# FrancisGregoryNg/Gaussian_Process_Optimization

Hardware: AMD Instinct MI355X
Metric: GP fit+predict iters/sec at N=16384 D=8 (higher is better)
Workload: dtype f64; 1 GPU; C3 (BASELINE.json configs[2]): N=16384, D=8 RBF iso, fit (K, Cholesky, alpha, LML) + predict mean/var at M=10000 candidates + EI arg-best; candidates_total=10000, candidates_this_rank=10000, entry_point=gp_fit_predict, kernel=RBF, fit=replicated on every rank (does not shard, SURVEY.md 8e), torch_imported=False, launcher=single process, emulate_fp64=0

## Files before the change

### gaussian_process_optimization_amd/csrc/api_factor.hip

```cpp
#include "api_internal.h"

void build_ky(gp_ctx *g, const Members &m, bool jittered) {
    launch_kbuild(g->s, m.A, m.lda, m.X, g->N, g->Npad, m.kp[0], m.diag[0], 0, m.nb, m.sA, m.kpt, m.diag_tab, m.sX);
    if (jittered) launch_add_diag(g->s, m.A, m.lda, g->N, m.jit[0], m.nb, m.sA, m.jit_tab);
    launch_set_rhs(g->s, m.A, m.lda, m.Y, g->N, g->Npad, g->P, m.nb, m.sA, m.sY);
}

static int chain_step(gp_ctx *g, hipStream_t s, const Members &m, int j, int J1, int R1) {
    double *A = m.A, *invL = m.invL;
    const long lda = m.lda;
    if (g->inner_tiles >= 2 && m.nb == 1 && j + 1 < J1 && R1 - (j + 2) >= g->inner_min_rows) {
        launch_potrf_pair(s, A, lda, j, invL, m.info);
        launch_trsm2(s, A, lda, j, invL, j + 2, R1);
        if (j + 2 < J1)
            gemm(g, s, 1, A, lda, A + (long)j * GP_TILE, lda, A + (long)j * GP_TILE, lda, 1, 2 * GP_TILE,
                 TileSet{0, R1, j + 2, J1, 1});
        return j + 2;
    }
    launch_potrf_tile(s, A, lda, j, invL, m.info, m.nb, m.sA, m.sI, 4);
    gemm(g, s, 0, A, lda, A + (long)j * GP_TILE, lda, invL + (long)j * GP_TILE * GP_TILE, GP_TILE, 0, GP_TILE,
         TileSet{j + 1, R1, j, j + 1, 0}, member_opt(m, inplace_opt(), m.sA, m.sA, m.sI));
    if (j + 1 < J1)
        gemm(g, s, 1, A, lda, A + (long)j * GP_TILE, lda, A + (long)j * GP_TILE, lda, 1, GP_TILE, TileSet{0, R1, j + 1, J1, 1},
             member_opt(m, GemmOpt(), m.sA, m.sA, m.sA));
// ... 126 lines not shown
        if (Gf == 1) {
            rlaunch(sb, J, J1, J2, p.nt, J == 0 ? 1 : 0);
            rebuild_next(J);
            GP_NOTE(hipEventRecord(la_event(g, EV_BULK, J), sb));
            return;
        }
        const int gi = J / Gf, Jg = gi * Gf;
        const int first = gi == 0 ? 1 : 0;
        GP_NOTE(hipEventRecord(la_event(g, EV_CONV, J), sb));
        rlaunch(sb, Jg, J1, p.edge(J + 2), p.edge(J + 3), first);
        rebuild_next(J);
        GP_NOTE(hipEventRecord(la_event(g, EV_BULK, J), sb));
        if (J % Gf == Gf - 1) {
            if (gi >= 1 && far_issued[gi - 1]) GP_NOTE(hipStreamWaitEvent(sb, la_event(g, EV_FAR, gi - 1), 0));
            mid_Jg = Jg;
            mid_end = J1;
            mid_first = first;
            mid_base = J + 3;
            mid_next = 0;
            if (p.edge(J + 3 + Gf) < p.nt) {
                GP_NOTE(hipStreamWaitEvent(sfar, la_event(g, EV_CONV, J), 0));
                rlaunch(sfar, Jg, J1, p.edge(J + 3 + Gf), p.nt, first);
                GP_NOTE(hipEventRecord(la_event(g, EV_FAR, gi), sfar));
                far_issued[gi] = true;
            }
        }
        if (mid_Jg >= 0 && mid_next < Gf) {
            rlaunch(sb, mid_Jg, mid_end, p.edge(mid_base + mid_next), p.edge(mid_base + mid_next + 1), mid_first);
            ++mid_next;
        }
    }
};

int factor_lookahead(gp_ctx *g, const PredPipe &pp) {
    int rc;
    if ((rc = ensure_bulk_stream(g))) return rc;
    const LaPlan p = la_plan(g, pp);
    const int nt = p.nt;
    hipStream_t sp = g->s_panel, sb = g->s_bulk;
    hipStream_t spred = pp.on ? g->s_pred : nullptr, sfar = p.Gf > 1 ? g->s_pred : nullptr;
    if ((rc = reserve_panel_inv(g, p.W, nt))) return rc;
    Members cm = ctx_members(g);
    cm.W = p.W;
    record_wait(g, EV_MISC, 0, g->s, {sp, sb, g->s_inv, spred, sfar});
    if (pp.on && pp.init) pp.init(spred);
    EmuTrail emu{g, p, cm};
    if (p.emu && (rc = emu.prepare())) return rc;
    int next_pred = 0;
    int own_prev = nt;
    for (int J = 0; J < p.nJ; ++J) {
        const int J0 = p.pb[J], J1 = p.pb[J + 1], J2 = p.pb[J + 2];
        for (int j = J0; j < J1;) j = chain_step(g, sp, cm, j, J1, p.R1);
        record_wait(g, EV_CHAIN, J, sp, {g->s_inv});
        build_panel_inv_one(g, g->s_inv, J, p.W, nt);
        if (J < p.pstages) GP_NOTE(hipEventRecord(la_event(g, EV_INVP, J), g->s_inv));
        if (pp.on && J >= p.pred_start) release_stages(g, p, pp, cm, J, &next_pred);
        if (J1 >= nt) break;
        const int oc = p.emu ? nt : first_owned_column(nt, J2, p.W, own_prev, g->own_keep_base, g->own_keep_per_row,
                                                       g->own_keep_pipe_pct, pp.on && J >= p.pred_start);
        own_prev = nt - oc;
        if (oc < nt && J >= 1) panel_update(g, sp, cm, J0, J1, TileSet{0, p.R1, oc, nt, 1});
        if (J >= 1) GP_NOTE(hipStreamWaitEvent(sp, la_event(g, EV_BULK, J - 1), 0));
        panel_update(g, sp, cm, J0, J1, TileSet{0, p.R1, J1, J2, 1});
        if (oc < nt && J == 0)
            panel_update(g, sp, cm, J0, J1, TileSet{0, p.R1, oc, nt, 1});
        if (J2 >= nt) continue;
        GP_NOTE(hipStreamWaitEvent(sb, la_event(g, EV_CHAIN, J), 0));
        if (p.emu) emu.update(J);
        else trail_fp64(g, p, cm, J, oc);
    }
    record_wait(g, EV_MISC, 1, sp, {g->s});
    record_wait(g, EV_MISC, 2, sb, {g->s});
    if (sfar) record_wait(g, EV_MISC, 7, sfar, {g->s});
    g->pipe_done = p.pstages;
    if (spred) record_wait(g, EV_MISC, 3, spred, {g->s});
    record_wait(g, EV_MISC, 4, g->s_inv, {g->s});
    g->invp_W = p.W;
    g->invp_valid = true;
    return la_events_ok(g);
}

__device__ __forceinline__ void dot_ay_body(const double *alpha, long lda_, const double *Y, long N, int P, double *out) {
    __shared__ double sh[16];
    const int p = blockIdx.x;
    double s = 0.0;
    for (long i = threadIdx.x; i < N; i += 1024) s = fma(alpha[p * lda_ + i], Y[i * P + p], s);
    for (int o = 32; o > 0; o >>= 1) s += __shfl_down(s, o);
    if ((threadIdx.x & 63) == 0) sh[threadIdx.x >> 6] = s;
    __syncthreads();
    if (threadIdx.x == 0) {
        double r = 0.0;
        for (int i = 0; i < 16; ++i) r += sh[i];
        out[p] = r;
    }
}

__global__ void dot_ay_kernel(const double *alpha, long lda_, const double *Y, long N, int P, double *out) {
    dot_ay_body(alpha, lda_, Y, N, P, out);
}
__global__ void dot_ay_batch_kernel(const double *alpha, long sV, long lda_, const double *Y, long sY, long N, int P, double *out,
// ... 114 lines not shown
    if ((rc = g->dT2.reserve(mcpad * Npad))) return rc;
    if (!cand && (rc = g->dWi.reserve(Npad * Npad))) return rc;
    if ((rc = reserve_panel_inv(g, W, nt))) return rc;
    pp->on = true;
    pp->mt = (int)(mcpad / GP_TILE);
    pp->nJ = nJ;
    pp->trapezoid = !cand;
    if (cand) {
        pp->init = [g, mcpad, N, Npad](hipStream_t st) { launch_cross_k(st, g->dT, Npad, g->dXs, g->M, mcpad, g->dX, N, Npad, g->kp); };
        pp->phase = "cholesky+cand_solve";
        pp->rest_phase = "cand_solve_rest";
        pp->flops = (double)N * N * N / 3.0 + (double)N * N * g->M;
        pp->stages = g->pipe_stages;
        if (pp->stages <= 0) pp->stages = std::max(1, (nJ * 14 + 50) / 100) + (nJ <= 12 ? 1 : 0);
        pp->start_pct = g->pipe_start_pct;
        if (pp->start_pct < 0) pp->start_pct = nJ <= 24 ? 32 : 40;
    } else {
        pp->init = [g, Npad](hipStream_t st) { launch_set_identity(st, g->dT, Npad, Npad); };
        pp->phase = "cholesky+potri_stages";
        pp->rest_phase = "potri_solve_rest";
        pp->flops = (double)N * N * N / 3.0;
        pp->stages = g->pipe_stages_grad;
        if (pp->stages <= 0) pp->stages = std::max(1, (nJ * 36 + 50) / 100);
        pp->start_pct = g->pipe_start_pct_grad;
    }
    return 0;
}

static int factor_attempt(gp_ctx *g, const PredPipe &pp, const double *diag_add, const double *jitter) {
    const double N = (double)g->N;
    const int nt = (int)(g->Npad / GP_TILE);
    g->lr_valid = false;
    g->jitter_try = *jitter;
    int ph = phase_begin(g, "kbuild", 0.0, 8.0 * N * g->D + 8.0 * N * N / 2);
    Members m = ctx_members(g);
    m.diag = diag_add;
    m.jit = jitter;
    build_ky(g, m, *jitter != 0.0);
    phase_end(g, ph);
    HIPCHK(hipMemsetAsync(g->dInfo, 0, sizeof(int) * 4, g->s));
    ph = phase_begin(g, pp.on ? pp.phase : "cholesky", pp.on ? pp.flops : N * N * N / 3.0, 0.0);
    const bool la = pp.on || (g->lookahead && nt > g->panel_tiles && (nt > g->lookahead_min_tiles || emu_fit_applies(g)));
    const int rc = la ? factor_lookahead(g, pp) : factor(g);
    if (rc) return rc;
    phase_end(g, ph);
    return 0;
}

static int rest_stages(gp_ctx *g, const PredPipe &pp, bool *side_alpha) {
    if (g->pipe_done >= pp.nJ) return 0;
    const int phr = phase_begin(g, pp.rest_phase, 0.0, 0.0);
    const int rci = ensure_panel_inv(g);
    if (rci) return rci;
    *side_alpha = g->s_inv && g->side_alpha;
    hipEvent_t eI = la_event(g, EV_MISC, 5);
    if (*side_alpha) GP_NOTE(hipEventRecord(eI, g->s));
    solve_rows(g, ctx_members(g), pp.mt, pp.trapezoid, g->pipe_done);
    if (*side_alpha) {
        GP_NOTE(hipStreamWaitEvent(g->s_inv, eI, 0));
        alpha_lml(g, g->s_inv, ctx_members(g));
        GP_NOTE(hipEventRecord(la_event(g, EV_MISC, 6), g->s_inv));
    }
    phase_end(g, phr);
    return 0;
}

int fit_impl(gp_ctx *g, int maxtries, Pipe kind, int include_noise) {
    HIPCHK(hipSetDevice(g->device));
    QuiesceOnError guard{g};
    const long N = g->N, Npad = g->Npad;
    const int P = g->P;
    int rc;
    if ((rc = mean_residuals(g))) return rc;
    PredPipe pp;
    if (kind != Pipe::None && (rc = make_pipe(g, kind, &pp))) return rc;
    double diag_add, diag0;
    ky_diag(g->kp, g->noise, &diag_add, &diag0);
    g->nphases = 0;
    g->emu_off_call = false;
    fit_dropped(g);

    double jitter = 0.0;
    int tries = 0;
    for (int info = 0, bad = 0;;) {
        if ((rc = factor_attempt(g, pp, &diag_add, &jitter))) return rc;
        if ((rc = factor_status(g, g->emulate_fp64 && !g->emu_off_call, &info, &bad))) return rc;
        if (bad) {
            g->emu_off_call = true;
            ++g->emu_fallbacks;
            g->nphases = 0;
            g->invp_valid = false;
            continue;
        }
        if (info == 0) break;
        g->invp_valid = false;
        const int rcl = ladder_step(diag0, maxtries, info, &jitter, &tries);
        if (rcl == GP_ERR_NOT_PD_DIAG) return fail(rcl, "not pd: non-positive diagonal elements");
        if (rcl) {
            g_err = "not positive definite, even with jitter.";
            return rcl;
        }
        g->nphases = 0;
    }
    g->jitter = jitter;

    bool side_alpha = false;
    if (pp.on && (rc = rest_stages(g, pp, &side_alpha))) return rc;
    if (kind == Pipe::Identity) {
        if ((rc = wi_lauum(g))) return rc;
        g->wi_valid = true;
        g->w_in_t2 = true;
    }
    int ph = phase_begin(g, "alpha_lml", 2.0 * (double)N * N * P, 8.0 * (double)N * N / 2);
    if (side_alpha) {
        GP_NOTE(hipStreamWaitEvent(g->s, la_event(g, EV_MISC, 6), 0));
    } else {
        if ((rc = ensure_panel_inv(g))) return rc;
        alpha_lml(g, g->s, ctx_members(g));
    }
    phase_end(g, ph);
    if (kind == Pipe::Candidates) {
        ph = phase_begin(g, "reduce", 0.0, 8.0 * (double)N * g->M);
        launch_predict_reduce(g->s, g->dT2, Npad, g->M, N, g->dA + Npad * Npad, Npad, P, g->kp.variance,
                              include_noise ? g->noise : 0.0, g->dMean, g->dVar);
        mean_add(g, g->dXs, g->M, g->dMean);
        phase_end(g, ph);
    }

    std::vector<double> sc(SCAL_DOT.off + P);
    HIPCHK(hipMemcpyAsync(sc.data(), g->dScal, sizeof(double) * sc.size(), hipMemcpyDeviceToHost, g->s));
    GP_SYNC(g->s);
    g->logdet = sc[SCAL_LOGDET.off];
    g->lml = lml_from_scalars(N, P, sc.data());
    g->fitted = true;
    if (kind == Pipe::Candidates) {
        g->predicted = true;
        g->predicted_noise = include_noise ? 1 : 0;
    }
    guard.armed = false;
    return 0;
}

extern "C" int gp_fit(gp_t *g, int maxtries, double *lml, double *logdet, double *jitter_used) {
    if (!g) return fail(GP_ERR_ARG, "null gp");
    GP_DEAD_CHECK(g);
    if (!g->have_data || !g->have_params) return fail(GP_ERR_STATE, "set data and params before gp_fit");
    int rc = fit_impl(g, maxtries, Pipe::None, 0);
    if (rc) return rc;
    if (lml) *lml = g->lml;
    if (logdet) *logdet = g->logdet;
    if (jitter_used) *jitter_used = g->jitter;
    return 0;
}

extern "C" int gp_fit_predict(gp_t *g, int maxtries, int include_noise, double *lml, double *logdet, double *jitter_used,
                   double *mean, double *var) {
    if (!g) return fail(GP_ERR_ARG, "null gp");
    GP_DEAD_CHECK(g);
    if (!g->have_data || !g->have_params) return fail(GP_ERR_STATE, "set data and params before gp_fit_predict");
    if (g->M < 1) return fail(GP_ERR_STATE, "gp_set_candidates first");
    HIPCHK(hipSetDevice(g->device));
    const int nt = (int)(g->Npad / GP_TILE);
    const bool can_pipe = g->lookahead && nt > g->panel_tiles && round_up(g->M, GP_TILE) <= g->mc_max && !g->emulate_fp64 &&
                          g->M > g->small_m;
    int rc;
    if (can_pipe) {
        if ((rc = fit_impl(g, maxtries, Pipe::Candidates, include_noise))) return rc;
    } else {
        if ((rc = fit_impl(g, maxtries, Pipe::None, 0))) return rc;
        if ((rc = ensure_out(g))) return rc;
        if ((rc = run_predict(g, include_noise))) return rc;
    }
    if (lml) *lml = g->lml;
    if (logdet) *logdet = g->logdet;
    if (jitter_used) *jitter_used = g->jitter;
    if (mean) HIPCHK(hipMemcpyAsync(mean, g->dMean, sizeof(double) * g->M * g->P, hipMemcpyDeviceToHost, g->s));
    if (var) HIPCHK(hipMemcpyAsync(var, g->dVar, sizeof(double) * g->M, hipMemcpyDeviceToHost, g->s));
    GP_SYNC(g->s);
    return 0;
}
```

### gaussian_process_optimization_amd/csrc/api_internal.h

```cpp
#pragma once
#include "gphip_internal.h"
#include "warp_math.h"
#include "../../include/gphip.h"

#include <hip/hip_ext.h>
#include <rccl/rccl.h>

#include <algorithm>
#include <array>
#include <cmath>
#include <cstdarg>
#include <cstdio>
#include <cstdlib>
#include <cstring>
#include <functional>
#include <map>
#include <mutex>
#include <set>
#include <string>
#include <type_traits>
#include <vector>

extern thread_local std::string g_err;
int fail(int code, const char *fmt, ...);
// ... 42 lines not shown
    } while (0)

struct Slot { long off, len; };
template <size_t n>
constexpr bool slots_ok(const Slot (&s)[n], long cap) {
    for (size_t i = 0; i < n; ++i) {
        if (s[i].off < 0 || s[i].len < 1 || s[i].off + s[i].len > cap) return false;
        for (size_t j = 0; j < i; ++j)
            if (s[i].off < s[j].off + s[j].len && s[j].off < s[i].off + s[i].len) return false;
    }
    return true;
}
#define GP_GRAD_MAX_P 16
#define GP_LP_MAX_NB 256
#define GP_EXCLUDE_MAX 256
#define GP_COMM_MAX_RANKS 128
constexpr long SCAL_CAP = 512;
constexpr Slot SCAL_LOGDET{0, 1};
constexpr Slot SCAL_DOT{8, GP_MAX_RHS};
constexpr Slot SCAL_DOT_GRAD{8, GP_GRAD_MAX_P};
constexpr Slot SCAL_GRAD{64, GP_MAX_D / GP_GRAD_CH * GP_GRAD_NACC};
constexpr Slot SCAL_FIT_RECORD{400, 4};
constexpr Slot SCAL_TRACE{420, 2};
constexpr Slot SCAL_WARP_LOGJAC{430, 1};
constexpr Slot SCAL_WARP_GRAD{431, GP_WARP_NPSI};
static_assert(GP_MAX_D % GP_GRAD_CH == 0, "whole gradient passes");
static_assert(slots_ok({SCAL_LOGDET, SCAL_DOT, SCAL_FIT_RECORD, SCAL_TRACE}, SCAL_CAP), "dScal: a fit of up to GP_MAX_RHS outputs");
static_assert(slots_ok({SCAL_LOGDET, SCAL_DOT_GRAD, SCAL_GRAD, SCAL_FIT_RECORD, SCAL_TRACE}, SCAL_CAP), "dScal: fit and gradient");
static_assert(slots_ok({SCAL_LOGDET, SCAL_DOT_GRAD, SCAL_GRAD, SCAL_FIT_RECORD, SCAL_TRACE, SCAL_WARP_LOGJAC, SCAL_WARP_GRAD}, SCAL_CAP),
              "dScal: fit and gradient of a warped model (gp_fit_grad_warp)");
constexpr long REDV_CAP = 512, REDI_CAP = 1024;
constexpr Slot RED_PARTIAL{0, 256};
constexpr Slot RED_RESULT{256, 1};
constexpr Slot REDV_GATHER_SEND{300, 2};
constexpr Slot REDV_GATHER_RECV{304, 200};
constexpr Slot REDI_EXCLUDE{300, GP_EXCLUDE_MAX};
static_assert(slots_ok({RED_PARTIAL, RED_RESULT, REDV_GATHER_SEND, REDV_GATHER_RECV}, REDV_CAP), "dRedV");
static_assert(slots_ok({RED_PARTIAL, RED_RESULT, REDI_EXCLUDE}, REDI_CAP), "dRedI");
constexpr long COMM_CAP = 2L * GP_TOPK_MAX * (1 + GP_COMM_MAX_RANKS);
constexpr Slot COMM_TOPK_VAL{0, GP_TOPK_MAX}, COMM_TOPK_ROW{GP_TOPK_MAX, GP_TOPK_MAX};
constexpr Slot COMM_SEND{0, 2 * GP_TOPK_MAX}, COMM_RECV{2 * GP_TOPK_MAX, 2L * GP_TOPK_MAX * GP_COMM_MAX_RANKS};
static_assert(slots_ok({COMM_TOPK_VAL, COMM_TOPK_ROW}, COMM_CAP), "dComm: gp_acq_topk");
static_assert(slots_ok({COMM_SEND, COMM_RECV}, COMM_CAP), "dComm: gathers");
constexpr long LP_CAP = (long)GP_LP_MAX_NB * (GP_MAX_D + 2);
constexpr Slot LP_X{0, (long)GP_LP_MAX_NB * GP_MAX_D}, LP_R{LP_X.off + LP_X.len, GP_LP_MAX_NB}, LP_S{LP_R.off + LP_R.len, GP_LP_MAX_NB};
static_assert(slots_ok({LP_X, LP_R, LP_S}, LP_CAP), "dLp");

struct Phase {
    const char *name;
    hipEvent_t e0, e1;
    double flops, bytes;
    bool used;
};
#define MAX_PHASES 16

template <class T>
struct DevBuf {
    T *p = nullptr;
    long cap = 0;
    DevBuf() = default;
    DevBuf(DevBuf &&o) noexcept : p(o.p), cap(o.cap) { o.p = nullptr; o.cap = 0; }
    DevBuf(const DevBuf &) = delete;
    DevBuf &operator=(const DevBuf &) = delete;
    ~DevBuf() { release(); }
    operator T *() const { return p; }
    void release() {
        if (p) (void)hipFree(p);
        p = nullptr;
        cap = 0;
    }
    hipError_t alloc(long n) {
// ... 192 lines not shown
    DevBuf<double> dMu;
    DevBuf<int> dInfo;
    DevBuf<double> dScal;
    DevBuf<double> dRedV;
    DevBuf<long long> dRedI;
    long capN = 0;
    int capP = 0;
    KernParams kp{};
    int ard = 0;
    double noise = 0.0;
    bool have_data = false, have_params = false;
    double jitter = 0.0, lml = 0.0, logdet = 0.0;
    double fmin = 0.0;
    bool fitted = false;
    bool fmin_valid = false;
    bool wi_valid = false;
    bool li_valid = false;
    long rows_calls_since_fit = 0;
    bool w_in_t2 = false;
    bool invp_valid = false;
    bool lr_valid = false;
    bool predicted = false;
    int cost_tab = 0;
    long M = 0;
    DevBuf<double> dXs;
    DevBuf<double> dT;
    DevBuf<double> dMean, dVar, dAcq;
    int predicted_noise = -1;
    DevBuf<double> dWi;
    DevBuf<double> dT2;
    DevBuf<double> dLi;
    DevBuf<double> dRows;
    PassOwner pass{1, "the one-location kernels"};
    std::vector<double> lp_cache;
    int lp_cache_nb = -1;
    long rows_fused_calls = 0, rows_fallback_calls = 0;
    long rows_narrow_passes = 0, rows_wide_passes = 0;
    int rows_wide = 1;
    int rows_build = -1;
    int rows_nt = -1;
    DevBuf<double> dLp;
    DevBuf<double> dApp;
    long append_in_place = 0, append_relayout = 0, append_refused = 0;
    DevBuf<double> dX2, dK2;
    DevBuf<double> dCov;
    DevBuf<double> dInvP, dInvPw;
    int invp_W = 0;
    DevBuf<double> dDm, dDv, dDacq;
    int panel_tiles = 6;
    int lookahead = 1;
    int inner_min_rows = 0;
    int own_keep_per_row = 36, own_keep_base = 200;
    int own_keep_pipe_pct = 0;
    int inner_tiles = 1;
    int lookahead_min_tiles = 40;
    int reserve_cus = 32;
    long mc_max = 16384;
    long small_m = 8;
    Phase phases[MAX_PHASES];
    int nphases = 0;
    bool profiling = false;
    int profile_class = 0;
    std::vector<hipEvent_t> gemm_events;
    std::vector<hipEvent_t> rns_events;
    size_t rns_ev_used = 0;
    double rns_ops = 0.0;
// ... 198 lines not shown
    bool trapezoid = false;
    int eS = -1;
    signed char *Wr = nullptr;
    long wpitch = 0, wplane = 0;
};

struct DevStreams {
    hipStream_t s = nullptr, panel = nullptr, bulk = nullptr, inv = nullptr, pred = nullptr;
    int reserved = -1;
};

enum { EV_CHAIN = 0, EV_BULK = 1, EV_INVP = 2, EV_MISC = 3, EV_FAR = 4, EV_CONV = 5 };

void shutdown_all();
int sparse_fitted(gp_ctx *g);
int make_bulk_stream(int device, int reserve, hipStream_t *out);
int get_streams(int device, int reserve, DevStreams *out);
int phase_begin(gp_ctx *g, const char *name, double flops, double bytes);
void phase_end(gp_ctx *g, int id);
void gemm(gp_ctx *g, hipStream_t s, int mode, double *C, long ldc, const double *A, long lda, const double *B, long ldb, int b_mul, int K, TileSet ts, const GemmOpt &o = GemmOpt());
void rns_gemm(gp_ctx *g, hipStream_t s, const signed char *A, long lda, long a_plane, const signed char *B, long ldb, long b_plane, signed char *R, int mt_all, int nt_all, int mt, int c0, int c1, int K, int first, int tri = 0);
void destroy_ctx_events(gp_ctx *g);
void build_ky(gp_ctx *g, const Members &m, bool jittered);
void factor_buf(gp_ctx *g, const Members &m, int nt, int R1, bool side_inv = false);
int factor(gp_ctx *g);
void alpha_lml(gp_ctx *g, hipStream_t s, const Members &m);
void ky_diag(const KernParams &kp, double noise, double *diag_add, double *diag0);
int ladder_step(double diag0, int maxtries, int info, double *jitter, int *tries);
int factor_status(gp_ctx *g, bool emu, int *info, int *bad);
double lml_from_scalars(long N, int P, const double *scal);
void build_panel_inv_one(gp_ctx *g, hipStream_t s, int J, int W, int nt);
int rns_prepare(gp_ctx *g, double jitter, RnsGeom *r);
void rns_convert_panel(gp_ctx *g, hipStream_t s, const RnsGeom &r, int J, int *flag);
int factor_lookahead(gp_ctx *g, const PredPipe &pp = PredPipe());
int ensure_bulk_stream(gp_ctx *g);
hipEvent_t la_event(gp_ctx *g, int kind, size_t i);
int la_events_ok(gp_ctx *g);
int reserve_panel_inv(gp_ctx *g, int W, int nt);
int ensure_panel_inv(gp_ctx *g);
void identity_blocks(hipStream_t s, double *T, long n, int nb);
void panel_inv_members(gp_ctx *g, const Members &m);
void solve_step(gp_ctx *g, hipStream_t s, const Members &m, int J, int rows);
void solve_rows(gp_ctx *g, const Members &m, int mt, int trapezoid, int J_from = 0);
int solve_rows_rns(gp_ctx *g, double *T, double *S, int mt, const RnsSolveOpt &opt = RnsSolveOpt());
int fit_impl(gp_ctx *g, int maxtries, Pipe kind, int include_noise);
using ChunkHook = std::function<int(long, long, long)>;
int run_predict(gp_ctx *g, int include_noise, bool tiles_only = false, const ChunkHook *chunk = nullptr);
int ensure_out(gp_ctx *g);
struct AcqSpec { int type; double par, fmin, y_mean, y_std; bool feas_ok = false; bool mes_ok = false; const double *mes_y = nullptr; int mes_K = 0; };
struct LpSpec { int transform; const double *Xb; int nb; const double *r0, *s0; };
static inline int acq_base(int type) { return type & ~GP_ACQ_PER_COST; }
static inline bool acq_per_cost(int type) { return (type & GP_ACQ_PER_COST) != 0; }
static inline bool acq_times_feas(const AcqSpec &a) { return a.feas_ok && (a.type & GP_ACQ_TIMES_FEAS) != 0; }
static inline int acq_rule(const AcqSpec &a) { return acq_base(a.feas_ok ? a.type & ~GP_ACQ_TIMES_FEAS : a.type); }
static inline AcqSpec exact_spec(const gp_ctx *g, AcqSpec a) {
    a.mes_ok = true;
    if (g) {
        a.mes_y = g->mes.dY.p;
        a.mes_K = g->mes.K;
    }
    return a;
}
int check_acq(const gp_ctx *g, const AcqSpec &a, const LpSpec *lp = nullptr);
int check_per_cost(const gp_ctx *g, int type, bool lp);
int cost_divide(gp_ctx *g, const double *X, long M, bool grad, double *acq, double *dacq);
void cost_divide_block(gp_ctx *g, const RowsX &rx, bool grad, double *blk, int MV);
void feas_apply(gp_ctx *g, bool pof, double *acq);
int train_values(gp_ctx *g);
bool rows_take_fused(gp_ctx *g, int64_t M);
int rows_prepare(gp_ctx *g);
void rows_enqueue(gp_ctx *g, const RowsX &rx, int include_noise, int want_grad, const RowsAcq &aq, PassReport *r, unsigned *arrivals);
int check_lp(const LpSpec &lp);
int check_sense(int sense);
int check_k(int k);
int check_exclude(const int64_t *exclude, int nex, int64_t M);
int argbest_read(gp_ctx *g, const double *v, long n, int sense, int64_t *idx, double *val);
struct ScoreRows { const double *X; long M; const double *mean, *var, *dm, *dv; double *acq, *dacq; };
int score_rows(gp_ctx *g, const AcqSpec &a, const LpSpec *lp, bool grad, const ScoreRows &r);
int select_best(gp_ctx *g, double *scores, long M, int sense, const int64_t *exclude, int nex, int64_t *idx, double *val);
int select_topk(gp_ctx *g, double *scores, long M, int sense, int k, int64_t *idx, double *val);
int scores_out(gp_ctx *g, const double *acq, const double *dacq, long M, int D, double *out, double *dout);
static inline double acq_empty(int sense) { return sense > 0 ? -INFINITY : INFINITY; }
struct LpBatch { double *X = nullptr, *r = nullptr, *s = nullptr; };
static inline LpBatch lp_slots(const gp_ctx *g) { return LpBatch{g->dLp + LP_X.off, g->dLp + LP_R.off, g->dLp + LP_S.off}; }
RowsAcq rows_acq(const AcqSpec &a, const LpSpec *lp, const LpBatch &b);
int run_acq(gp_ctx *g, const AcqSpec &a, const LpSpec *lp, bool grad);
int upload_lp_batch(gp_ctx *g, const LpSpec &lp, LpBatch *b);
int rows_lp_batch(gp_ctx *g, const LpSpec &lp, LpBatch *b);
int acq_values(gp_ctx *g, const AcqSpec &a, const LpSpec *lp, double *out, double *dout);
int acq_argbest(gp_ctx *g, const AcqSpec &a, const LpSpec *lp, int sense, const int64_t *exclude, int nex, int64_t *idx, double *val);
int acq_topk(gp_ctx *g, const AcqSpec &a, int sense, int k, int64_t *idx, double *val);
void pack_pairs(const double *v, const int64_t *ix, size_t n, double *rec);
void unpack_pairs(const double *rec, size_t n, double *v, int64_t *ix);
void lauum(gp_ctx *g, const Members &m);
int wi_lauum(gp_ctx *g);
int wi_rns(gp_ctx *g);
int ensure_wi(gp_ctx *g);
int ensure_linv(gp_ctx *g);
int lml_grad_lds_check(const gp_ctx *g, const char *who);
int gradx_lds_check(const gp_ctx *g, const char *who);
void lml_grad_passes(gp_ctx *g, const Members &m);
// ... 17 lines not shown
```

### gaussian_process_optimization_amd/csrc/api_predict.hip

```cpp
#include "api_internal.h"

extern "C" int gp_set_candidates(gp_t *g, const double *Xs, int64_t M) {
    if (!g || !Xs) return fail(GP_ERR_ARG, "null argument");
    GP_DEAD_CHECK(g);
    if (!g->have_data) return fail(GP_ERR_STATE, "gp_set_data first");
    if (M < 1) return fail(GP_ERR_ARG, "M < 1");
    HIPCHK(hipSetDevice(g->device));
    GP_SYNC(g->s);
    int rc;
    if ((rc = g->dXs.reserve((long)M * g->D))) return rc;
    HIPCHK(hipMemcpy(g->dXs, Xs, sizeof(double) * M * g->D, hipMemcpyHostToDevice));
    g->M = M;
    g->predicted = false;
    if (g->cost_tab == 1) g->cost_tab = 0;
    g->feas.K = 0;
    return 0;
}

extern "C" int gp_set_candidates_kumar(gp_t *g, const double *Xs, int64_t M, const int *warp, const double *a, const double *b,
                                       const double *xmin, const double *xmax, double *warped_out) {
    if (!g || !Xs || !warp || !a || !b || !xmin || !xmax) return fail(GP_ERR_ARG, "null argument");
    GP_DEAD_CHECK(g);
    if (!g->have_data) return fail(GP_ERR_STATE, "gp_set_data first");
    GP_NO_MEAN(g, "gp_set_candidates_kumar");
// ... 194 lines not shown
    const int kk = (int)std::min<long>(k, M);
    for (int j = 0; j < kk; ++j) {
        argbest_launch(g, scores, M, sense);
        HIPCHK(hipMemcpyAsync(dv + j, g->dRedV + RED_RESULT.off, 8, hipMemcpyDeviceToDevice, g->s));
        HIPCHK(hipMemcpyAsync(di + j, g->dRedI + RED_RESULT.off, 8, hipMemcpyDeviceToDevice, g->s));
        launch_mask(g->s, scores, g->dRedI + RED_RESULT.off, 1, acq_empty(sense));
    }
    std::vector<long long> hi(kk);
    HIPCHK(hipMemcpyAsync(val, dv, sizeof(double) * kk, hipMemcpyDeviceToHost, g->s));
    HIPCHK(hipMemcpyAsync(hi.data(), di, sizeof(long long) * kk, hipMemcpyDeviceToHost, g->s));
    GP_SYNC(g->s);
    for (int j = 0; j < kk; ++j) idx[j] = (int64_t)hi[j];
    for (int j = kk; j < k; ++j) {
        idx[j] = -1;
        val[j] = acq_empty(sense);
    }
    return 0;
}

int scores_out(gp_ctx *g, const double *acq, const double *dacq, long M, int D, double *out, double *dout) {
    if (out) HIPCHK(hipMemcpyAsync(out, acq, sizeof(double) * M, hipMemcpyDeviceToHost, g->s));
    if (dout) HIPCHK(hipMemcpyAsync(dout, dacq, sizeof(double) * M * D, hipMemcpyDeviceToHost, g->s));
    GP_SYNC(g->s);
    return 0;
}

int train_values(gp_ctx *g) {
    if (g->fmin_direct) {
        launch_train_mean(g->s, g->dX, g->N, g->kp, g->dAlpha, g->dMu);
        mean_add(g, g->dX, g->N, g->dMu);
    } else {
        launch_train_mean_identity(g->s, g->mean.on() ? g->dYraw : g->dY, g->dAlpha, g->noise + 1e-8 + g->jitter, g->N, g->dMu);
    }
    return 0;
}

extern "C" int gp_fmin(gp_t *g, double *fmin) {
    if (!g || !fmin) return fail(GP_ERR_ARG, "null argument");
    GP_FITTED(g);
    if (g->P != 1) return fail(GP_ERR_ARG, "gp_fmin needs P == 1");
    if (!g->fmin_valid) {
        int rc;
        if ((rc = train_values(g))) return rc;
        if ((rc = argbest_read(g, g->dMu, g->N, -1, nullptr, &g->fmin))) return rc;
        g->fmin_valid = true;
    }
    *fmin = g->fmin;
    return 0;
}

int run_acq(gp_ctx *g, const AcqSpec &a, const LpSpec *lp, bool grad) {
    int rc;
    if (lp && (rc = check_lp(*lp))) return rc;
    if ((rc = check_acq(g, a, lp))) return rc;
    if ((rc = ensure_out(g))) return rc;
    if (grad && (rc = run_predict_grad(g))) return rc;
    if (!g->predicted || g->predicted_noise != 1)
        if ((rc = run_predict(g, 1))) return rc;
    return score_rows(g, a, lp, grad, ScoreRows{g->dXs, g->M, g->dMean, g->dVar, g->dDm, g->dDv, g->dAcq, g->dDacq});
}

extern "C" int gp_acq(gp_t *g, int type, double par, double fmin, double y_mean, double y_std, double *out) {
    if (!g || !out) return fail(GP_ERR_ARG, "null argument");
    GP_SCORING(g);
    return acq_values(g, exact_spec(g, AcqSpec{type, par, fmin, y_mean, y_std, true}), nullptr, out, nullptr);
}
// ... 140 lines not shown
```

### gaussian_process_optimization_amd/csrc/gphip_internal.h

```cpp
#pragma once
#include <hip/hip_runtime.h>
#include <stdint.h>
#include <algorithm>
#include <string>
#include <vector>

#define GP_TILE 128
#define GP_MAX_RHS 128

typedef double double4_t __attribute__((ext_vector_type(4)));
typedef double double2_t __attribute__((ext_vector_type(2)));

void gp_note_hip(hipError_t e, const char *what, const char *file, int line);
#define GP_NOTE(call) gp_note_hip((call), #call, __FILE__, __LINE__)
#define GP_LAUNCH(kernel, grid, block, lds, stream, ...)                                   \
    do {                                                                                   \
        (void)hipGetLastError();  \
        hipLaunchKernelGGL(kernel, grid, block, lds, stream, __VA_ARGS__);                 \
        gp_note_hip(hipGetLastError(), #kernel, __FILE__, __LINE__);                       \
    } while (0)

#define GP_MAX_D 64
struct KernParams {
    int kernel;
// ... 88 lines not shown
    return n;
}

struct GemmOpt {
    int k_tri = 0;
    int k_sub = 0;
    int k_end_tri = 0;
    int b_sub = 0;
    int batch = 1;
    int members = 1;
    long sC = 0, sA = 0, sB = 0;
    const short *tile_list = nullptr;
    int stagger = 0;
    int small = 0;
    int waves8 = 0;
    int sched = 0;
    int inplace = 0;
    int rows64 = 0;
    int pair = 0;
};
std::vector<short> build_tile_list(const TileSet &ts, int S);
void launch_gemm_nt(hipStream_t s, int mode, double *C, long ldc, const double *A, long lda,
                    const double *B, long ldb, int b_mul, int K, TileSet ts, const GemmOpt &o = GemmOpt());

void launch_potrf_tile(hipStream_t s, double *A, long lda, int t, double *invL, int *info, int nb = 1, long sA = 0, long sI = 0,
                       int sInfo = 0);
void launch_potrf_pair(hipStream_t s, double *A, long lda, int t, double *invL, int *info);
void launch_trsm2(hipStream_t s, double *A, long lda, int t, const double *invL, int r0, int r1);
void potrf_set_debug_lds(int bytes);


void launch_kbuild(hipStream_t s, double *A, long lda, const double *X, long N, long Npad, const KernParams &kp, double diag_add,
                   int full, int nb = 1, long sA = 0, const KernParams *kpt = nullptr, const double *diag_tab = nullptr, long sX = 0);
void launch_set_rhs(hipStream_t s, double *A, long lda, const double *Y, long N, long Npad, int P, int nb = 1, long sA = 0, long sY = 0);
void launch_cross_k(hipStream_t s, double *T, long ldt, const double *Xs, long M, long Mpad,
                    const double *X, long N, long Npad, const KernParams &kp, int nb = 1, long sT = 0, long sX = 0,
                    const KernParams *kpt = nullptr);

void launch_cross_k_rows(hipStream_t s, double *T, long ldt, const double *Xs, int M, const double *X, long N, long Npad,
                         const KernParams &kp);

void launch_logdet(hipStream_t s, const double *A, long lda, long N, double *out, int nb = 1, long sA = 0, long so = 0);
void launch_rhs_sumsq(hipStream_t s, const double *A, long lda, long N, long Npad, int P, double *out);

void launch_trsv_backward(hipStream_t s, const double *L, long lda, const double *invP, int W, long Npad, const double *Z, long ldz,
                          int P, double *Aout, double *w, int nb = 1, long sL = 0, long sP = 0, long sV = 0);

void launch_predict_reduce(hipStream_t s, const double *T, long ldt, long M, long N, const double *Z,
                           long ldz, int P, double kss, double noise_add, double *mean, double *var);

void launch_train_mean(hipStream_t s, const double *X, long N, const KernParams &kp, const double *alpha,
                       double *mu);
void launch_train_mean_identity(hipStream_t s, const double *Y, const double *alpha, double d, long N, double *mu);
void launch_min(hipStream_t s, const double *v, long n, double *out);

void launch_acq(hipStream_t s, int type, double par, double fmin, double y_mean, double y_std,
                const double *mean, const double *var, long M, double *out);
void launch_argbest(hipStream_t s, const double *v, long n, int sense, double *best_val, long long *best_idx,
                    double *scratch_val, long long *scratch_idx);

void launch_mes_acq(hipStream_t s, const double *ystar, int K, double y_mean, double y_std, const double *mean, const double *var,
                    const double *dmdx, const double *dvdx, long M, int D, double *out, double *dout);
#define MES_CHUNK 256
#define MES_MAX_G 64
struct MesY {
    int G;
// ... 245 lines not shown
```

### gaussian_process_optimization_amd/csrc/kbuild.hip

```cpp
#include "gphip_internal.h"

#define k_of_r2 gp_k_of_r2
template <int FP>
__device__ __forceinline__ double gower_factor_pair(int kernel, double variance, double dx, int disc) {
    const double r = disc ? (dx != 0.0 ? 1.0 : 0.0) : fabs(dx);
    return gp_k_of_r2_pair<FP>(kernel, variance, r * r);
}
__device__ __forceinline__ double gower_factor(int kernel, double variance, double dx, int disc) {
    return gower_factor_pair<0>(kernel, variance, dx, disc);
}

__device__ __forceinline__ void stage_rows_T(double *dst, const double *X, long row0, long N, int D,
                                             const double *ls, int tid) {
    for (int idx = tid; idx < GP_TILE * D; idx += 256) {
        const int r = idx / D, d = idx - r * D;
        const long g = row0 + r;
        dst[d * GP_TILE + r] = (g < N) ? X[g * D + d] / ls[d] : 0.0;
    }
}

template <int DU, int FP>
__device__ __forceinline__ void kbuild_body(double *A, long lda, const double *X, long N, long Npad, const KernParams &kp,
                                            double diag_add, int full, int nt) {
    extern __shared__ __attribute__((aligned(16))) double sm[];
    const int DS = DU > 0 ? DU : kp.D;
    double *xi = sm;
    double *xj = sm + (long)DS * GP_TILE;
    __shared__ double ils[GP_MAX_D];
    const int tid = threadIdx.x;
    int tm, tn;
    if (full) {
        tm = blockIdx.x / nt;
        tn = blockIdx.x % nt;
    } else {
        const long t = blockIdx.x;
        tm = (int)((sqrt(8.0 * (double)t + 1.0) - 1.0) * 0.5);
        while ((long)tm * (tm + 1) / 2 > t) --tm;
        while ((long)(tm + 1) * (tm + 2) / 2 <= t) ++tm;
        tn = (int)(t - (long)tm * (tm + 1) / 2);
    }
    if (tid < kp.D) ils[tid] = kp_div(kp, tid);
    __syncthreads();
    stage_rows_T(xi, X, (long)tm * GP_TILE, N, kp.D, ils, tid);
    stage_rows_T(xj, X, (long)tn * GP_TILE, N, kp.D, ils, tid);
    if (DU > 0)
        for (int idx = kp.D * GP_TILE + tid; idx < DU * GP_TILE; idx += 256) xi[idx] = xj[idx] = 0.0;
    __syncthreads();

    const int cx = (tid & 63) * 2;
    const int ry = tid >> 6;
    const long gc = (long)tn * GP_TILE + cx;
    double2_t bq[DU > 0 ? DU : 1];
    if (DU > 0) {
#pragma unroll
        for (int d = 0; d < DU; ++d) bq[d] = *(const double2_t *)(xj + d * GP_TILE + cx);
    }
    for (int q = 0; q < 32; ++q) {
        const int r = ry + 4 * q;
        const long gr = (long)tm * GP_TILE + r;
        double2_t out;
        if (kp.gower) {
            double p0 = 1.0, p1 = 1.0;
            for (int d = 0; d < kp.D; ++d) {
                const double a = xi[d * GP_TILE + r];
                const double2_t b = *(const double2_t *)(xj + d * GP_TILE + cx);
                p0 *= gower_factor_pair<FP>(kp.kernel, kp.variance, a - b[0], kp.gdisc[d]);
                p1 *= gower_factor_pair<FP>(kp.kernel, kp.variance, a - b[1], kp.gdisc[d]);
            }
            out[0] = p0;
            out[1] = p1;
        } else {
// ... 3 lines not shown
                for (int d = 0; d < DU; ++d) {
                    const double a = xi[d * GP_TILE + r];
                    const double d0 = a - bq[d][0], d1 = a - bq[d][1];
                    s0 = fma(d0, d0, s0);
                    s1 = fma(d1, d1, s1);
                }
            } else {
                for (int d = 0; d < kp.D; ++d) {
                    const double a = xi[d * GP_TILE + r];
                    const double2_t b = *(const double2_t *)(xj + d * GP_TILE + cx);
                    const double d0 = a - b[0], d1 = a - b[1];
                    s0 = fma(d0, d0, s0);
                    s1 = fma(d1, d1, s1);
                }
            }
            out[0] = gp_k_of_r2_pair<FP>(kp.kernel, kp.variance, s0);
            out[1] = gp_k_of_r2_pair<FP>(kp.kernel, kp.variance, s1);
        }
        if (gr >= N) {
            out[0] = (gr == gc) ? 1.0 : 0.0;
            out[1] = (gr == gc + 1) ? 1.0 : 0.0;
        } else {
            if (gc >= N) out[0] = 0.0;
            else if (gr == gc) out[0] = (kp.gower ? out[0] : kp.variance) + diag_add;
            if (gc + 1 >= N) out[1] = 0.0;
            else if (gr == gc + 1) out[1] = (kp.gower ? out[1] : kp.variance) + diag_add;
        }
        *(double2_t *)(A + gr * lda + gc) = out;
    }
}

template <int DU, int FP>
__global__ __launch_bounds__(256) void kbuild_kernel(double *A, long lda, const double *X, long N, long Npad,
                                                     KernParams kp, double diag_add, int full, int nt) {
    kbuild_body<DU, FP>(A, lda, X, N, Npad, kp, diag_add, full, nt);
}
template <int DU, int FP>
__global__ __launch_bounds__(256) void kbuild_batch_kernel(double *A, long lda, long sA, const double *X, long sX, long N, long Npad,
                                                           const KernParams *kpt, const double *diag_add, int nt) {
    const long z = blockIdx.z;
    kbuild_body<DU, FP>(A + z * sA, lda, X + z * sX, N, Npad, kpt[z], diag_add[z], 0, nt);
}

static void launch_kbuild_members(hipStream_t s, double *A, long lda, long sA, const double *X, long sX, long N, long Npad, int DU, int fp,
                                  size_t shm, const KernParams *kpt, const double *diag_tab, int nb);
#define KB_LAUNCH_PAIR(kernel, DU, fp, ...)                       \
    do {                                                          \
        if (fp) GP_LAUNCH((kernel<DU, 1>), __VA_ARGS__);          \
        else GP_LAUNCH((kernel<DU, 0>), __VA_ARGS__);             \
    } while (0)

void launch_kbuild(hipStream_t s, double *A, long lda, const double *X, long N, long Npad, const KernParams &kp, double diag_add,
                   int full, int nb, long sA, const KernParams *kpt, const double *diag_tab, long sX) {
    const int nt = (int)(Npad / GP_TILE);
    const long nblk = full ? (long)nt * nt : (long)nt * (nt + 1) / 2;
    const int DU = kp.gower ? 0 : (kp.D <= 8 ? 8 : (kp.D <= 16 ? 16 : 0));
    const size_t shm = (size_t)2 * (DU ? DU : kp.D) * GP_TILE * sizeof(double);
    const int fp = GP_FAMILY_PAIR(kp.kernel);
    if (nb > 1) return launch_kbuild_members(s, A, lda, sA, X, sX, N, Npad, DU, fp, shm, kpt, diag_tab, nb);
    if (DU == 8)
        KB_LAUNCH_PAIR(kbuild_kernel, 8, fp, dim3((unsigned)nblk), dim3(256), shm, s, A, lda, X, N, Npad, kp, diag_add, full, nt);
    else if (DU == 16)
        KB_LAUNCH_PAIR(kbuild_kernel, 16, fp, dim3((unsigned)nblk), dim3(256), shm, s, A, lda, X, N, Npad, kp, diag_add, full, nt);
    else
        KB_LAUNCH_PAIR(kbuild_kernel, 0, fp, dim3((unsigned)nblk), dim3(256), shm, s, A, lda, X, N, Npad, kp, diag_add, full, nt);
}

__device__ __forceinline__ void set_rhs_body(double *A, long lda, const double *Y, long N, long Npad, int P) {
    const long i = (long)blockIdx.x * blockDim.x + threadIdx.x;
    const int p = blockIdx.y;
    if (i >= Npad) return;
    A[(Npad + p) * lda + i] = (p < P && i < N) ? Y[i * P + p] : 0.0;
}
__global__ void set_rhs_kernel(double *A, long lda, const double *Y, long N, long Npad, int P) {
    set_rhs_body(A, lda, Y, N, Npad, P);
}
__global__ void set_rhs_batch_kernel(double *A, long lda, long sA, const double *Y, long sY, long N, long Npad, int P) {
    set_rhs_body(A + (long)blockIdx.z * sA, lda, Y + (long)blockIdx.z * sY, N, Npad, P);
}

void launch_set_rhs(hipStream_t s, double *A, long lda, const double *Y, long N, long Npad, int P, int nb, long sA, long sY) {
    if (nb > 1) {
        dim3 grid((unsigned)((Npad + 255) / 256), GP_MAX_RHS, (unsigned)nb);
        GP_LAUNCH(set_rhs_batch_kernel, grid, dim3(256), 0, s, A, lda, sA, Y, sY, N, Npad, P);
        return;
    }
    dim3 grid((unsigned)((Npad + 255) / 256), GP_MAX_RHS);
    GP_LAUNCH(set_rhs_kernel, grid, dim3(256), 0, s, A, lda, Y, N, Npad, P);
}

template <int DU, int FP>
__device__ __forceinline__ void cross_k_body(double *T, long ldt, const double *Xs, long M, const double *X, long N,
                                             const KernParams &kp, int nti) {
    extern __shared__ __attribute__((aligned(16))) double sm[];
    const int DS = DU > 0 ? DU : kp.D;
    double *xc = sm;
    double *xt = sm + (long)DS * GP_TILE;
    __shared__ double ils[GP_MAX_D];
// ... 148 lines not shown
```

Measured before the change: 14.97 fit+predict iters/s.

## Build first kernel-matrix panel ahead and overlap rest with Cholesky

When lookahead factorization runs without jitter, the kernel-matrix build is split by tile columns. The first panel columns are built before factorization starts, and the remaining columns are enqueued on the main stream so they overlap with the first panel's Cholesky chain, with event waits before the trailing updates. The fit also computes the training-set minimum (fmin) up front and copies scalars, fmin, mean and variance into one pinned host buffer with a single sync, which removes separate device-to-host copies and syncs. This adds column-ordered tile indexing in the kbuild kernel and extra event dependencies that must be correct for ordering.

```diff
diff --git a/gaussian_process_optimization_amd/csrc/api_factor.hip b/gaussian_process_optimization_amd/csrc/api_factor.hip
--- a/gaussian_process_optimization_amd/csrc/api_factor.hip
+++ b/gaussian_process_optimization_amd/csrc/api_factor.hip
@@ -182,7 +182,7 @@
     }
 };
 
-int factor_lookahead(gp_ctx *g, const PredPipe &pp) {
+int factor_lookahead(gp_ctx *g, const PredPipe &pp, const std::function<void()> *rest_of_ky) {
     int rc;
     if ((rc = ensure_bulk_stream(g))) return rc;
     const LaPlan p = la_plan(g, pp);
@@ -193,6 +193,10 @@
     Members cm = ctx_members(g);
     cm.W = p.W;
     record_wait(g, EV_MISC, 0, g->s, {sp, sb, g->s_inv, spred, sfar});
+    if (rest_of_ky) {
+        (*rest_of_ky)();
+        GP_NOTE(hipEventRecord(la_event(g, EV_MISC, 8), g->s));
+    }
     if (pp.on && pp.init) pp.init(spred);
     EmuTrail emu{g, p, cm};
     if (p.emu && (rc = emu.prepare())) return rc;
@@ -211,11 +215,13 @@
         own_prev = nt - oc;
         if (oc < nt && J >= 1) panel_update(g, sp, cm, J0, J1, TileSet{0, p.R1, oc, nt, 1});
         if (J >= 1) GP_NOTE(hipStreamWaitEvent(sp, la_event(g, EV_BULK, J - 1), 0));
+        if (J == 0 && rest_of_ky) GP_NOTE(hipStreamWaitEvent(sp, la_event(g, EV_MISC, 8), 0));
         panel_update(g, sp, cm, J0, J1, TileSet{0, p.R1, J1, J2, 1});
         if (oc < nt && J == 0)
             panel_update(g, sp, cm, J0, J1, TileSet{0, p.R1, oc, nt, 1});
         if (J2 >= nt) continue;
         GP_NOTE(hipStreamWaitEvent(sb, la_event(g, EV_CHAIN, J), 0));
+        if (J == 0 && rest_of_ky) GP_NOTE(hipStreamWaitEvent(sb, la_event(g, EV_MISC, 8), 0));
         if (p.emu) emu.update(J);
         else trail_fp64(g, p, cm, J, oc);
     }
@@ -396,16 +402,27 @@
     const int nt = (int)(g->Npad / GP_TILE);
     g->lr_valid = false;
     g->jitter_try = *jitter;
-    int ph = phase_begin(g, "kbuild", 0.0, 8.0 * N * g->D + 8.0 * N * N / 2);
+    const bool la = pp.on || (g->lookahead && nt > g->panel_tiles && (nt > g->lookahead_min_tiles || emu_fit_applies(g)));
+    const bool panel_order = la && *jitter == 0.0 && !emu_fit_applies(g);
+    const int phk = phase_begin(g, "kbuild", 0.0, 8.0 * N * g->D + 8.0 * N * N / 2);
     Members m = ctx_members(g);
     m.diag = diag_add;
     m.jit = jitter;
-    build_ky(g, m, *jitter != 0.0);
-    phase_end(g, ph);
-    HIPCHK(hipMemsetAsync(g->dInfo, 0, sizeof(int) * 4, g->s));
-    ph = phase_begin(g, pp.on ? pp.phase : "cholesky", pp.on ? pp.flops : N * N * N / 3.0, 0.0);
-    const bool la = pp.on || (g->lookahead && nt > g->panel_tiles && (nt > g->lookahead_min_tiles || emu_fit_applies(g)));
-    const int rc = la ? factor_lookahead(g, pp) : factor(g);
+    if (panel_order) {
+        HIPCHK(hipMemsetAsync(g->dInfo, 0, sizeof(int) * 4, g->s));
+        launch_set_rhs(g->s, m.A, m.lda, m.Y, g->N, g->Npad, g->P);
+        launch_kbuild_cols(g->s, m.A, m.lda, m.X, g->N, g->Npad, m.kp[0], m.diag[0], 0, g->panel_tiles);
+    } else {
+        build_ky(g, m, *jitter != 0.0);
+        phase_end(g, phk);
+        HIPCHK(hipMemsetAsync(g->dInfo, 0, sizeof(int) * 4, g->s));
+    }
+    const int ph = phase_begin(g, pp.on ? pp.phase : "cholesky", pp.on ? pp.flops : N * N * N / 3.0, 0.0);
+    const std::function<void()> rest_of_ky = [&] {
+        launch_kbuild_cols(g->s, m.A, m.lda, m.X, g->N, g->Npad, m.kp[0], m.diag[0], g->panel_tiles, nt);
+        phase_end(g, phk);
+    };
+    const int rc = la ? factor_lookahead(g, pp, panel_order ? &rest_of_ky : nullptr) : factor(g);
     if (rc) return rc;
     phase_end(g, ph);
     return 0;
@@ -429,12 +446,14 @@
     return 0;
 }
 
-int fit_impl(gp_ctx *g, int maxtries, Pipe kind, int include_noise) {
+int fit_impl(gp_ctx *g, int maxtries, Pipe kind, int include_noise, double *mean_out, double *var_out) {
     HIPCHK(hipSetDevice(g->device));
     QuiesceOnError guard{g};
     const long N = g->N, Npad = g->Npad;
     const int P = g->P;
     int rc;
+    const long n_mean = mean_out ? g->M * P : 0, n_var = var_out ? g->M : 0;
+    if ((rc = g->pin.reserve(PIN_POST.off + n_mean + n_var))) return rc;
     if ((rc = mean_residuals(g))) return rc;
     PredPipe pp;
     if (kind != Pipe::None && (rc = make_pipe(g, kind, &pp))) return rc;
@@ -491,16 +510,28 @@
         phase_end(g, ph);
     }
 
-    std::vector<double> sc(SCAL_DOT.off + P);
-    HIPCHK(hipMemcpyAsync(sc.data(), g->dScal, sizeof(double) * sc.size(), hipMemcpyDeviceToHost, g->s));
+    const bool eager_fmin = kind == Pipe::Candidates && P == 1 && !g->fmin_direct;
+    if (eager_fmin && (rc = fmin_enqueue(g))) return rc;
+
+    double *pin = g->pin.p, *sc = pin + PIN_SCAL.off, *pmean = pin + PIN_POST.off, *pvar = pmean + n_mean;
+    HIPCHK(hipMemcpyAsync(sc, g->dScal, sizeof(double) * (SCAL_DOT.off + P), hipMemcpyDeviceToHost, g->s));
+    if (eager_fmin) HIPCHK(hipMemcpyAsync(pin + PIN_FMIN.off, g->dRedV + RED_FMIN.off, sizeof(double), hipMemcpyDeviceToHost, g->s));
+    if (n_mean) HIPCHK(hipMemcpyAsync(pmean, g->dMean, sizeof(double) * n_mean, hipMemcpyDeviceToHost, g->s));
+    if (n_var) HIPCHK(hipMemcpyAsync(pvar, g->dVar, sizeof(double) * n_var, hipMemcpyDeviceToHost, g->s));
     GP_SYNC(g->s);
     g->logdet = sc[SCAL_LOGDET.off];
-    g->lml = lml_from_scalars(N, P, sc.data());
+    g->lml = lml_from_scalars(N, P, sc);
     g->fitted = true;
     if (kind == Pipe::Candidates) {
         g->predicted = true;
         g->predicted_noise = include_noise ? 1 : 0;
     }
+    if (eager_fmin) {
+        g->fmin = pin[PIN_FMIN.off];
+        g->fmin_valid = true;
+    }
+    if (n_mean) memcpy(mean_out, pmean, sizeof(double) * n_mean);
+    if (n_var) memcpy(var_out, pvar, sizeof(double) * n_var);
     guard.armed = false;
     return 0;
 }
@@ -529,17 +560,17 @@
                           g->M > g->small_m;
     int rc;
     if (can_pipe) {
-        if ((rc = fit_impl(g, maxtries, Pipe::Candidates, include_noise))) return rc;
+        if ((rc = fit_impl(g, maxtries, Pipe::Candidates, include_noise, mean, var))) return rc;
     } else {
         if ((rc = fit_impl(g, maxtries, Pipe::None, 0))) return rc;
         if ((rc = ensure_out(g))) return rc;
         if ((rc = run_predict(g, include_noise))) return rc;
+        if (mean) HIPCHK(hipMemcpyAsync(mean, g->dMean, sizeof(double) * g->M * g->P, hipMemcpyDeviceToHost, g->s));
+        if (var) HIPCHK(hipMemcpyAsync(var, g->dVar, sizeof(double) * g->M, hipMemcpyDeviceToHost, g->s));
+        GP_SYNC(g->s);
     }
     if (lml) *lml = g->lml;
     if (logdet) *logdet = g->logdet;
     if (jitter_used) *jitter_used = g->jitter;
-    if (mean) HIPCHK(hipMemcpyAsync(mean, g->dMean, sizeof(double) * g->M * g->P, hipMemcpyDeviceToHost, g->s));
-    if (var) HIPCHK(hipMemcpyAsync(var, g->dVar, sizeof(double) * g->M, hipMemcpyDeviceToHost, g->s));
-    GP_SYNC(g->s);
-    return 0;
-}
+    return 0;
+}
diff --git a/gaussian_process_optimization_amd/csrc/api_internal.h b/gaussian_process_optimization_amd/csrc/api_internal.h
--- a/gaussian_process_optimization_amd/csrc/api_internal.h
+++ b/gaussian_process_optimization_amd/csrc/api_internal.h
@@ -98,11 +98,16 @@
 constexpr long REDV_CAP = 512, REDI_CAP = 1024;
 constexpr Slot RED_PARTIAL{0, 256};
 constexpr Slot RED_RESULT{256, 1};
+constexpr Slot RED_FMIN{257, 1};
 constexpr Slot REDV_GATHER_SEND{300, 2};
 constexpr Slot REDV_GATHER_RECV{304, 200};
 constexpr Slot REDI_EXCLUDE{300, GP_EXCLUDE_MAX};
-static_assert(slots_ok({RED_PARTIAL, RED_RESULT, REDV_GATHER_SEND, REDV_GATHER_RECV}, REDV_CAP), "dRedV");
-static_assert(slots_ok({RED_PARTIAL, RED_RESULT, REDI_EXCLUDE}, REDI_CAP), "dRedI");
+static_assert(slots_ok({RED_PARTIAL, RED_RESULT, RED_FMIN, REDV_GATHER_SEND, REDV_GATHER_RECV}, REDV_CAP), "dRedV");
+static_assert(slots_ok({RED_PARTIAL, RED_RESULT, RED_FMIN, REDI_EXCLUDE}, REDI_CAP), "dRedI");
+constexpr Slot PIN_SCAL{0, SCAL_DOT.off + GP_MAX_RHS};
+constexpr Slot PIN_FMIN{PIN_SCAL.len, 1};
+constexpr Slot PIN_POST{PIN_SCAL.len + 8, 1};
+static_assert(slots_ok({PIN_SCAL, PIN_FMIN, PIN_POST}, PIN_POST.off + 1), "pin");
 constexpr long COMM_CAP = 2L * GP_TOPK_MAX * (1 + GP_COMM_MAX_RANKS);
 constexpr Slot COMM_TOPK_VAL{0, GP_TOPK_MAX}, COMM_TOPK_ROW{GP_TOPK_MAX, GP_TOPK_MAX};
 constexpr Slot COMM_SEND{0, 2 * GP_TOPK_MAX}, COMM_RECV{2 * GP_TOPK_MAX, 2L * GP_TOPK_MAX * GP_COMM_MAX_RANKS};
@@ -361,6 +366,7 @@
     DevBuf<double> dLi;
     DevBuf<double> dRows;
     PassOwner pass{1, "the one-location kernels"};
+    PinBuf pin;
     std::vector<double> lp_cache;
     int lp_cache_nb = -1;
     long rows_fused_calls = 0, rows_fallback_calls = 0;
@@ -625,7 +631,7 @@
 void build_panel_inv_one(gp_ctx *g, hipStream_t s, int J, int W, int nt);
 int rns_prepare(gp_ctx *g, double jitter, RnsGeom *r);
 void rns_convert_panel(gp_ctx *g, hipStream_t s, const RnsGeom &r, int J, int *flag);
-int factor_lookahead(gp_ctx *g, const PredPipe &pp = PredPipe());
+int factor_lookahead(gp_ctx *g, const PredPipe &pp = PredPipe(), const std::function<void()> *rest_of_ky = nullptr);
 int ensure_bulk_stream(gp_ctx *g);
 hipEvent_t la_event(gp_ctx *g, int kind, size_t i);
 int la_events_ok(gp_ctx *g);
@@ -636,7 +642,7 @@
 void solve_step(gp_ctx *g, hipStream_t s, const Members &m, int J, int rows);
 void solve_rows(gp_ctx *g, const Members &m, int mt, int trapezoid, int J_from = 0);
 int solve_rows_rns(gp_ctx *g, double *T, double *S, int mt, const RnsSolveOpt &opt = RnsSolveOpt());
-int fit_impl(gp_ctx *g, int maxtries, Pipe kind, int include_noise);
+int fit_impl(gp_ctx *g, int maxtries, Pipe kind, int include_noise, double *mean_out = nullptr, double *var_out = nullptr);
 using ChunkHook = std::function<int(long, long, long)>;
 int run_predict(gp_ctx *g, int include_noise, bool tiles_only = false, const ChunkHook *chunk = nullptr);
 int ensure_out(gp_ctx *g);
@@ -660,6 +666,7 @@
 void cost_divide_block(gp_ctx *g, const RowsX &rx, bool grad, double *blk, int MV);
 void feas_apply(gp_ctx *g, bool pof, double *acq);
 int train_values(gp_ctx *g);
+int fmin_enqueue(gp_ctx *g);
 bool rows_take_fused(gp_ctx *g, int64_t M);
 int rows_prepare(gp_ctx *g);
 void rows_enqueue(gp_ctx *g, const RowsX &rx, int include_noise, int want_grad, const RowsAcq &aq, PassReport *r, unsigned *arrivals);
diff --git a/gaussian_process_optimization_amd/csrc/api_predict.hip b/gaussian_process_optimization_amd/csrc/api_predict.hip
--- a/gaussian_process_optimization_amd/csrc/api_predict.hip
+++ b/gaussian_process_optimization_amd/csrc/api_predict.hip
@@ -250,6 +250,14 @@
     } else {
         launch_train_mean_identity(g->s, g->mean.on() ? g->dYraw : g->dY, g->dAlpha, g->noise + 1e-8 + g->jitter, g->N, g->dMu);
     }
+    return 0;
+}
+
+int fmin_enqueue(gp_ctx *g) {
+    int rc;
+    if ((rc = train_values(g))) return rc;
+    launch_argbest(g->s, g->dMu, g->N, -1, g->dRedV + RED_FMIN.off, g->dRedI + RED_FMIN.off, g->dRedV + RED_PARTIAL.off,
+                   g->dRedI + RED_PARTIAL.off);
     return 0;
 }
 
diff --git a/gaussian_process_optimization_amd/csrc/gphip_internal.h b/gaussian_process_optimization_amd/csrc/gphip_internal.h
--- a/gaussian_process_optimization_amd/csrc/gphip_internal.h
+++ b/gaussian_process_optimization_amd/csrc/gphip_internal.h
@@ -144,6 +144,8 @@
 
 void launch_kbuild(hipStream_t s, double *A, long lda, const double *X, long N, long Npad, const KernParams &kp, double diag_add,
                    int full, int nb = 1, long sA = 0, const KernParams *kpt = nullptr, const double *diag_tab = nullptr, long sX = 0);
+void launch_kbuild_cols(hipStream_t s, double *A, long lda, const double *X, long N, long Npad, const KernParams &kp, double diag_add,
+                        int c0, int c1);
 void launch_set_rhs(hipStream_t s, double *A, long lda, const double *Y, long N, long Npad, int P, int nb = 1, long sA = 0, long sY = 0);
 void launch_cross_k(hipStream_t s, double *T, long ldt, const double *Xs, long M, long Mpad,
                     const double *X, long N, long Npad, const KernParams &kp, int nb = 1, long sT = 0, long sX = 0,
diff --git a/gaussian_process_optimization_amd/csrc/kbuild.hip b/gaussian_process_optimization_amd/csrc/kbuild.hip
--- a/gaussian_process_optimization_amd/csrc/kbuild.hip
+++ b/gaussian_process_optimization_amd/csrc/kbuild.hip
@@ -19,9 +19,15 @@
     }
 }
 
+__device__ __forceinline__ int tri_row(long t) {
+    int tm = (int)((sqrt(8.0 * (double)t + 1.0) - 1.0) * 0.5);
+    while ((long)tm * (tm + 1) / 2 > t) --tm;
+    while ((long)(tm + 1) * (tm + 2) / 2 <= t) ++tm;
+    return tm;
+}
 template <int DU, int FP>
 __device__ __forceinline__ void kbuild_body(double *A, long lda, const double *X, long N, long Npad, const KernParams &kp,
-                                            double diag_add, int full, int nt) {
+                                            double diag_add, int full, int nt, long t0 = 0) {
     extern __shared__ __attribute__((aligned(16))) double sm[];
     const int DS = DU > 0 ? DU : kp.D;
     double *xi = sm;
@@ -29,14 +35,17 @@
     __shared__ double ils[GP_MAX_D];
     const int tid = threadIdx.x;
     int tm, tn;
-    if (full) {
+    if (full == 1) {
         tm = blockIdx.x / nt;
         tn = blockIdx.x % nt;
+    } else if (full == 2) {
+        const long u = (long)nt * (nt + 1) / 2 - 1 - (t0 + blockIdx.x);
+        const int a = tri_row(u);
+        tn = nt - 1 - a;
+        tm = nt - 1 - (int)(u - (long)a * (a + 1) / 2);
     } else {
         const long t = blockIdx.x;
-        tm = (int)((sqrt(8.0 * (double)t + 1.0) - 1.0) * 0.5);
-        while ((long)tm * (tm + 1) / 2 > t) --tm;
-        while ((long)(tm + 1) * (tm + 2) / 2 <= t) ++tm;
+        tm = tri_row(t);
         tn = (int)(t - (long)tm * (tm + 1) / 2);
     }
     if (tid < kp.D) ils[tid] = kp_div(kp, tid);
@@ -106,8 +115,8 @@
 
 template <int DU, int FP>
 __global__ __launch_bounds__(256) void kbuild_kernel(double *A, long lda, const double *X, long N, long Npad,
-                                                     KernParams kp, double diag_add, int full, int nt) {
-    kbuild_body<DU, FP>(A, lda, X, N, Npad, kp, diag_add, full, nt);
+                                                     KernParams kp, double diag_add, int full, int nt, long t0) {
+    kbuild_body<DU, FP>(A, lda, X, N, Npad, kp, diag_add, full, nt, t0);
 }
 template <int DU, int FP>
 __global__ __launch_bounds__(256) void kbuild_batch_kernel(double *A, long lda, long sA, const double *X, long sX, long N, long Npad,
@@ -124,20 +133,35 @@
         else GP_LAUNCH((kernel<DU, 0>), __VA_ARGS__);             \
     } while (0)
 
+static void launch_kbuild_one(hipStream_t s, double *A, long lda, const double *X, long N, long Npad, const KernParams &kp,
+                              double diag_add, int full, long nblk, long t0) {
+    const int nt = (int)(Npad / GP_TILE);
+    const int DU = kp.gower ? 0 : (kp.D <= 8 ? 8 : (kp.D <= 16 ? 16 : 0));
+    const size_t shm = (size_t)2 * (DU ? DU : kp.D) * GP_TILE * sizeof(double);
+    const int fp = GP_FAMILY_PAIR(kp.kernel);
+    if (DU == 8)
+        KB_LAUNCH_PAIR(kbuild_kernel, 8, fp, dim3((unsigned)nblk), dim3(256), shm, s, A, lda, X, N, Npad, kp, diag_add, full, nt, t0);
+    else if (DU == 16)
+        KB_LAUNCH_PAIR(kbuild_kernel, 16, fp, dim3((unsigned)nblk), dim3(256), shm, s, A, lda, X, N, Npad, kp, diag_add, full, nt, t0);
+    else
+        KB_LAUNCH_PAIR(kbuild_kernel, 0, fp, dim3((unsigned)nblk), dim3(256), shm, s, A, lda, X, N, Npad, kp, diag_add, full, nt, t0);
+}
 void launch_kbuild(hipStream_t s, double *A, long lda, const double *X, long N, long Npad, const KernParams &kp, double diag_add,
                    int full, int nb, long sA, const KernParams *kpt, const double *diag_tab, long sX) {
     const int nt = (int)(Npad / GP_TILE);
-    const long nblk = full ? (long)nt * nt : (long)nt * (nt + 1) / 2;
-    const int DU = kp.gower ? 0 : (kp.D <= 8 ? 8 : (kp.D <= 16 ? 16 : 0));
-    const size_t shm = (size_t)2 * (DU ? DU : kp.D) * GP_TILE * sizeof(double);
-    const int fp = GP_FAMILY_PAIR(kp.kernel);
-    if (nb > 1) return launch_kbuild_members(s, A, lda, sA, X, sX, N, Npad, DU, fp, shm, kpt, diag_tab, nb);
-    if (DU == 8)
-        KB_LAUNCH_PAIR(kbuild_kernel, 8, fp, dim3((unsigned)nblk), dim3(256), shm, s, A, lda, X, N, Npad, kp, diag_add, full, nt);
-    else if (DU == 16)
-        KB_LAUNCH_PAIR(kbuild_kernel, 16, fp, dim3((unsigned)nblk), dim3(256), shm, s, A, lda, X, N, Npad, kp, diag_add, full, nt);
-    else
-        KB_LAUNCH_PAIR(kbuild_kernel, 0, fp, dim3((unsigned)nblk), dim3(256), shm, s, A, lda, X, N, Npad, kp, diag_add, full, nt);
+    if (nb > 1) {
+        const int DU = kp.gower ? 0 : (kp.D <= 8 ? 8 : (kp.D <= 16 ? 16 : 0));
+        const size_t shm = (size_t)2 * (DU ? DU : kp.D) * GP_TILE * sizeof(double);
+        return launch_kbuild_members(s, A, lda, sA, X, sX, N, Npad, DU, GP_FAMILY_PAIR(kp.kernel), shm, kpt, diag_tab, nb);
+    }
+    launch_kbuild_one(s, A, lda, X, N, Npad, kp, diag_add, full ? 1 : 0, full ? (long)nt * nt : (long)nt * (nt + 1) / 2, 0);
+}
+void launch_kbuild_cols(hipStream_t s, double *A, long lda, const double *X, long N, long Npad, const KernParams &kp, double diag_add,
+                        int c0, int c1) {
+    const long nt = Npad / GP_TILE;
+    if (c0 < 0 || c1 > nt || c0 >= c1) return;
+    const long t0 = c0 * nt - (long)c0 * (c0 - 1) / 2, t1 = c1 * nt - (long)c1 * (c1 - 1) / 2;
+    launch_kbuild_one(s, A, lda, X, N, Npad, kp, diag_add, 2, t1 - t0, t0);
 }
 
 __device__ __forceinline__ void set_rhs_body(double *A, long lda, const double *Y, long N, long Npad, int P) {
```

New measurement: 15.05 fit+predict iters/s (median of 6 runs). Within noise of the previous version (+0.6%).
